# fatimp/SIFT3D

Hardware: AMD Instinct MI355X
Metric: Mvoxel/s detect+describe (float32 volume resident in HBM) (higher is better)
Workload: dtype f32; 1 GPU; 512x512x512 float32 lattice-blob volume, detect+describe, default parameters (sigma0 1.6, sigma_n 1.15, 3 levels/octave); parallelism=single GPU

## Files before the change

### include/sift3d_amd.h

```cpp
#ifndef SIFT3D_AMD_H
#define SIFT3D_AMD_H

#include <stddef.h>
#include <stdint.h>

#include "sift3d/imtypes.h"

#ifdef __cplusplus
extern "C" {
#endif

#define SIFT3D_AMD_API __attribute__((visibility("default")))


SIFT3D_AMD_API int
sift3d_amd_detect_keypoints_device(sift3d_detector *det, const float *d_volume,
                                   int nx, int ny, int nz, double ux, double uy,
                                   double uz, sift3d_keypoint_store *store);

SIFT3D_AMD_API int
sift3d_amd_image_set_units(sift3d_image *im, double ux, double uy, double uz);

SIFT3D_AMD_API int
sift3d_amd_detector_set_cuboid_extrema(sift3d_detector *det, int on);
// ... 813 lines not shown
    int32_t level;
    uint32_t row1;
    double sd;
} sift3d_hip_kp;

SIFT3D_AMD_API int
sift3d_hip_describe(const sift3d_hip_level *d_levels, const sift3d_hip_kp *d_kp,
                    uint32_t n, float *d_hist, void *stream);

SIFT3D_AMD_API size_t sift3d_hip_describe_wlut_floats(int nlevels);
SIFT3D_AMD_API int
sift3d_hip_describe_wlut(const sift3d_hip_level *d_levels, int nlevels, const sift3d_hip_kp *d_kp,
                         uint32_t n, float *d_hist, float *d_wlut, void *stream);
SIFT3D_AMD_API size_t sift3d_hip_describe_part_bytes(uint32_t n);
SIFT3D_AMD_API int
sift3d_hip_describe_parts(const sift3d_hip_level *d_levels, int nlevels, const sift3d_hip_kp *d_kp,
                          uint32_t n, uint32_t n_exact, float *d_hist, float *d_hist2, float *d_wlut,
                          void *d_part, void *stream);
SIFT3D_AMD_API int sift3d_hip_describe_lattice_level(float ux, float uy, float uz, double sd);
SIFT3D_AMD_API int
sift3d_hip_describe_lattice(const sift3d_hip_level *d_levels, int nlevels, const sift3d_hip_kp *d_kp,
                            uint32_t n, uint32_t n_exact, uint32_t n_lattice, float *d_hist, float *d_hist2,
                            float *d_wlut, void *d_part, void *stream);
SIFT3D_AMD_API int sift3d_hip_describe_addr32_level(const sift3d_hip_level *level, double sd);
SIFT3D_AMD_API int sift3d_hip_describe_addr32_records(const sift3d_hip_level *levels, int nlevels,
                                                      const sift3d_hip_kp *kp, uint32_t n);
SIFT3D_AMD_API int sift3d_hip_describe_addr_mode(int mode);
SIFT3D_AMD_API int
sift3d_hip_describe_lattice_a32(const sift3d_hip_level *d_levels, int nlevels, const sift3d_hip_kp *d_kp,
                                uint32_t n, uint32_t n_exact, uint32_t n_lattice, float *d_hist, float *d_hist2,
                                float *d_wlut, void *d_part, void *stream, int addr32);
SIFT3D_AMD_API int sift3d_hip_describe_rcp_check(uint32_t e_lo, uint32_t n_exp, uint64_t *mismatches,
                                                 uint32_t *first_bits, void *stream);
SIFT3D_AMD_API int
sift3d_hip_describe_clock(const float *d_wlut, int nlevels, int exact, uint64_t *cycles, uint64_t *ticks,
                          void *stream);
SIFT3D_AMD_API int
sift3d_hip_describe_wlut2(const sift3d_hip_level *d_levels, int nlevels, const sift3d_hip_kp *d_kp,
                          uint32_t n, float *d_hist, float *d_hist2, float *d_wlut, void *stream);
SIFT3D_AMD_API int
sift3d_hip_describe_ex(const sift3d_hip_level *d_levels, int nlevels, const sift3d_hip_kp *d_kp, uint32_t n,
                       uint32_t n_exact, float *d_hist, float *d_hist2, float *d_wlut, void *stream);

SIFT3D_AMD_API int sift3d_hip_slab_count(const sift3d_hip_cand *d_cand, const int32_t *d_keep, uint32_t n,
                                         int ngl, int K, int nkey, int32_t *d_cnt, void *stream);
SIFT3D_AMD_API size_t sift3d_hip_slab_pack_scratch_bytes(uint32_t n);
SIFT3D_AMD_API int sift3d_hip_slab_pack(const sift3d_hip_level *d_levels, const sift3d_hip_cand *d_cand,
                                        const int32_t *d_keep, const float *d_R, uint32_t n, int ngl,
                                        float *d_vals, void *d_recs, void *d_scratch, void *stream);
SIFT3D_AMD_API int sift3d_hip_slab_build(const void *d_all, size_t blk_bytes, size_t roff, size_t toff,
                                         int world, int nkey, const uint32_t *d_tab, uint32_t tot_k,
                                         uint32_t tot_c, void *d_out, void *stream);
typedef struct {
    size_t tot_c, tot_k;
    size_t maxc, maxk;
    size_t roff, toff, blk;
} sift3d_amd_slab_layout;
SIFT3D_AMD_API int sift3d_amd_slab_table(const void *cnt, size_t cnt_stride, int world, int nkey, uint32_t *tab,
                                         sift3d_amd_slab_layout *lay);

#define SIFT3D_HIP_FACE_FLOATS 19
SIFT3D_AMD_API int
sift3d_hip_set_mesh(const float *faces );

SIFT3D_AMD_API int
sift3d_hip_synth_lattice(float *d_dst, int nx, int ny, int nz, int z_off, uint64_t seed,
// ... 15 lines not shown
```

### profiles/describe_isa_cost.py

```python
#!/usr/bin/env python3
import argparse
import os
import re
import subprocess
import sys
import tempfile

HERE = os.path.dirname(os.path.abspath(__file__))
CSRC = os.path.join(HERE, "..", "sift3d_amd", "csrc")
RATES = os.path.join(HERE, "microbench", "valu_rate_mi355x.txt")
FLAGS = ["--offload-arch=gfx950", "-O3", "-ffp-contract=off", "-fPIC", "-std=c++17", "-fvisibility=hidden",
         "-fno-slp-vectorize", "--cuda-device-only", "-S", "-w"]
SUFFIXES = ("_e32", "_e64", "_dpp", "_sdwa", "_e64_dpp")
SALU_APART = ("s_waitcnt", "s_nop", "s_branch", "s_cbranch", "s_barrier", "s_endpgm", "s_sleep", "s_setprio")


def rates(path=RATES, waves=4):
    tab = {}
    for line in open(path):
        m = re.match(r"(\w+)\s+(\d+) waves/SIMD:.*->\s*([\d.]+) cycles", line)
        if m and int(m.group(2)) == waves:
            tab[m.group(1)] = float(m.group(3))
    return tab


def assembly(opt):
    with tempfile.TemporaryDirectory() as tmp:
        out = os.path.join(tmp, "describe.s")
        cmd = ["hipcc"] + FLAGS + ([] if opt is None else ["-DDESC_OPT=%d" % opt]) + ["sift3d_describe.hip", "-o", out]
        subprocess.run(cmd, cwd=CSRC, check=True)
        return open(out).read()


def kernel_body(text, instance):
    frag = "k_describeI" + "".join("Lb%dE" % (v.strip() == "true") for v in instance.split(",")) + "E"
    m = re.search(r"^(_Z\d+%s\w*):" % re.escape(frag), text, re.M)
    if not m:
        sys.exit("no instantiation %s in the assembly" % frag)
    end = text.index(".Lfunc_end", m.end())
    return m.group(1), text[m.end():end]


def base(op):
    for s in sorted(SUFFIXES, key=len, reverse=True):
        if op.endswith(s):
            return op[:-len(s)]
    return op


def blocks(body):
    out, cur = [], dict(label="entry", loop=None, depth=0, header=False, ops=[])
    for line in body.split("\n"):
        s = line.strip()
        m = re.match(r"(?:\.L(BB\d+_\d+)|; %bb\.(\d+)):\s*(?:;\s*(.*))?$", s)
        if m:
            out.append(cur)
            cur = dict(label=m.group(1) or "bb." + m.group(2), loop=None, depth=0, header=False, ops=[])
            note = m.group(3) or ""
            h = re.search(r"in Loop: Header=(BB\d+_\d+) Depth=(\d+)", note)
            if h:
                cur["loop"], cur["depth"] = h.group(1), int(h.group(2))
            elif "Loop Header" in note or "Parent Loop" in note:
                cur["header"] = True
            if re.search(r"This (Inner )?Loop Header: Depth=(\d+)", note):
                cur["header"], cur["loop"] = True, cur["label"]
                cur["depth"] = int(re.search(r"Depth=(\d+)", note).group(1))
            continue
        if cur["header"] and s.startswith(";"):
            h = re.search(r"This (?:Inner )?Loop Header: Depth=(\d+)", s)
            if h:
                cur["loop"], cur["depth"] = cur["label"], int(h.group(1))
            p = re.search(r"Parent Loop (BB\d+_\d+) Depth=(\d+)", s)
            if p:
                cur.setdefault("parents", []).append(p.group(1))
            continue
        if not s or s[0] in ";." or s.endswith(":"):
            continue
        cur["ops"].append(s.split()[0])
    out.append(cur)
    return out


def census(ops, tab, default):
    c = dict(valu=0, salu=0, lds=0, vmem=0, other=0, cycles=0.0)
    for op in ops:
        if op.startswith("v_"):
            c["valu"] += 1
            c["cycles"] += tab.get(base(op), default)
        elif op.startswith(SALU_APART):
            c["other"] += 1
        elif op.startswith("s_"):
            c["salu"] += 1
        elif op.startswith("ds_"):
            c["lds"] += 1
        elif op.startswith(("global_", "buffer_", "flat_")):
            c["vmem"] += 1
        else:
            c["other"] += 1
    return c


def row(name, c):
    return "%-22s %5d %5d %5d %5d %6d %9.0f" % (name, c["valu"], c["salu"], c["lds"], c["vmem"], c["other"], c["cycles"])


def add(cs):
    return {k: sum(c[k] for c in cs) for k in cs[0]}


def main():
    ap = argparse.ArgumentParser()
    ap.add_argument("--instance", default="false,true,false", help="template arguments of the instantiation")
    ap.add_argument("--opt", type=int, default=None, help="build with -DDESC_OPT=N")
    ap.add_argument("--asm", default=None, help="read this assembly file instead of compiling")
    ap.add_argument("--all", action="store_true", help="print every basic block")
    a = ap.parse_args()
    tab = rates()
    default = tab["v_fma_f32"]
    name, body = kernel_body(open(a.asm).read() if a.asm else assembly(a.opt), a.instance)
    bl = blocks(body)
    cs = [census(b["ops"], tab, default) for b in bl]
    print("# %s" % name)
    print("# VALU priced at 4 waves/SIMD (%s); opcodes not in the table: %.2f cycles" % (os.path.basename(RATES), default))
    print("%-22s %5s %5s %5s %5s %6s %9s" % ("block (loop, depth)", "VALU", "SALU", "LDS", "VMEM", "other", "VALU cyc"))
    for b, c in zip(bl, cs):
        if a.all or len(b["ops"]) >= 20:
            print(row("%s (%s, %d)" % (b["label"], b["loop"] or "-", b["depth"]), c))
    print(row("kernel", add(cs)))
    loops = {}
    for i, b in enumerate(bl):
        if b["loop"]:
            loops.setdefault(b["loop"], []).append(i)
    with_lds = [h for h, ix in loops.items() if sum(cs[i]["lds"] for i in ix) >= 32]
    if not with_lds:
        return
    batch_loop = max(with_lds, key=lambda h: max(len(bl[i]["ops"]) for i in loops[h]))
    big = sorted(sorted(loops[batch_loop], key=lambda i: -len(bl[i]["ops"]))[:2])
    print("# steady state of a batch (loop %s)" % batch_loop)
    for k, i in enumerate(big):
        print(row("pass %d = %s" % (k, bl[i]["label"]), cs[i]))
    print(row("both passes", add([cs[i] for i in big])))
    header = next(b for b in bl if b["label"] == batch_loop)
    parents = header.get("parents", [])
    if parents:
        scan = parents[-1]
        ix = [i for i in loops.get(scan, []) if bl[i]["loop"] == scan]
        print(row("scan iteration (%s)" % scan, add([cs[i] for i in ix])))


if __name__ == "__main__":
    main()
```

### sift3d_amd/csrc/sift3d_describe.hip

```cpp
#include "sift3d_kernels_common.h"
#include "sift3d_math.h"

#include <algorithm>
#include <cmath>
#include <cstdlib>

struct FaceRec {
    float v0[3], e1[3], e2[3], t[3], q[3], e2q, idx[3];
};
static_assert(sizeof(FaceRec) == SIFT3D_HIP_FACE_FLOATS * 4, "face record layout");

__constant__ float c_face16[20 * 16];
__constant__ int c_bin_off[12];
__constant__ int c_oct_face[32];

constexpr int DQ = 256;
constexpr int HIST_USED = 800;
constexpr int HIST_LDS = 800;
constexpr int FACE_STRIDE = 20;
constexpr int RSUPER = 68;
constexpr int REC_FLOATS = 7 * RSUPER;
constexpr int rec_row(int r) { return r < 7 ? r * RSUPER : (r - 7) * RSUPER + 32; }
constexpr int rec_group(int r) { return (rec_row(r) / 4) % 16; }
constexpr bool rec_groups_distinct()
// ... 13 lines not shown
}

#ifdef SIFT3D_AMD_DIAG
#define DESC_ABLATE_ARG , int ablate
#define DESC_ABLATE(bit) (ablate & (bit))
__device__ unsigned long long g_desc_voxels;
#else
#define DESC_ABLATE_ARG
#define DESC_ABLATE(bit) false
#endif

__device__ __forceinline__ void wave_sync()
{
    __builtin_amdgcn_fence(__ATOMIC_RELEASE, "wavefront");
    __builtin_amdgcn_wave_barrier();
    __builtin_amdgcn_fence(__ATOMIC_ACQUIRE, "wavefront");
}

__device__ __forceinline__ float quad_fmac(float acc, float x)
{
    asm("v_fmac_f32_dpp %0, %1, %1 quad_perm:[3,0,0,0] row_mask:0xf bank_mask:0xf bound_ctrl:1"
        : "+v"(acc)
        : "v"(x));
    return acc;
}

__device__ __forceinline__ float desc_rcp(float x)
{
    const float r = __builtin_amdgcn_rcpf(x);
    return __builtin_fmaf(r, __builtin_fmaf(-x, r, 1.0f), r);
}

__device__ __forceinline__ bool face_eval(const float4 *__restrict__ fr, float rx, float ry, float rz,
                                          float &xb, float &yb, float &zb, int &fi)
{
    const float4 A0 = fr[0], A1 = fr[1], A2 = fr[2], A3 = fr[3];
    const float px = ry * A1.y - rz * A1.x;
    const float py = rz * A0.w - rx * A1.y;
    const float pz = rx * A1.x - ry * A0.w;
    const float det = A0.x * px + A0.y * py + A0.z * pz;
    const float di = 1.0f / det;
    yb = di * (A1.z * px + A1.w * py + A2.x * pz);
    zb = di * (rx * A2.y + ry * A2.z + rz * A2.w);
    xb = 1.0f - yb - zb;
    const float kk = A3.x * di;
    fi = __float_as_int(A3.y);
    return !(fabsf(det) < 1.1920928955078125e-06f) &&
           !(xb < -1.1920928955078125e-06f || yb < -1.1920928955078125e-06f ||
             zb < -1.1920928955078125e-06f || kk < 0);
}

__device__ __forceinline__ int icos_guess(float rx, float ry, float rz)
{
    const float g = 1.6180339887f, g2 = 2.6180339887f;
    const float ax = fabsf(rx), ay = fabsf(ry), az = fabsf(rz);
    const float t1 = ax + g2 * ay - g * az;
    const float t2 = ay + g2 * az - g * ax;
    const float t3 = az + g2 * ax - g * ay;
    const int n1 = t1 < 0.0f, n2 = t2 < 0.0f, n3 = t3 < 0.0f;
    const int cls = n1 + (1 - n1) * (2 * n2 + (1 - n2) * 3 * n3);
    return cls * 8 + (int)(rx < 0.0f) + 2 * (int)(ry < 0.0f) + 4 * (int)(rz < 0.0f);
}

constexpr int WL_STRIDE = 4096, WL_HEAD = 4;
constexpr int WL_COUNTERS = 16;

__global__ __launch_bounds__(256) void k_desc_wlut(const sift3d_hip_level *__restrict__ levels, int nlevels,
                                                   float *__restrict__ lut)
{
    const int t = blockIdx.x;
    if (t >= nlevels)
        return;
    if (t == 0 && threadIdx.x < WL_COUNTERS)
        reinterpret_cast<uint32_t *>(lut + (size_t)nlevels * WL_STRIDE)[threadIdx.x] = 0u;
    const sift3d_hip_level L = levels[t];
    float *tab = lut + (size_t)t * WL_STRIDE;
    const float sigma = (float)(L.sd * 7.071067812);
    const float rad = (float)(2.0 * (double)sigma);
    const float rad2 = rad * rad, sig2 = sigma * sigma;
    int e;
    const float mant = frexpf(L.ux, &e);
    const float u2 = L.ux * L.ux;
    const bool ok = L.ux == L.uy && L.ux == L.uz && mant == 0.5f &&
                    rad2 / u2 < (float)(WL_STRIDE - WL_HEAD - 1) && u2 * (float)WL_STRIDE < 16777216.0f;
    if (threadIdx.x == 0) {
        tab[0] = ok ? 1.0f : 0.0f;
        tab[1] = 0.0f;
        tab[2] = __int_as_float((int)(__double_as_longlong(L.sd) & 0xffffffffll));
        tab[3] = __int_as_float((int)(__double_as_longlong(L.sd) >> 32));
    }
    if (!ok)
        return;
    for (int k = threadIdx.x; k < WL_STRIDE - WL_HEAD; k += 256) {
        const float sq = (float)k * u2;
        const float arg = -0.5f * sq / sig2;
        tab[WL_HEAD + k] = arg >= -150.0f ? s3d_expf(arg) : 0.0f;
    }
}

#ifndef DESC_OPT
#define DESC_OPT 495
#endif

constexpr int DWAVES = 4;
constexpr int DPARTS = 4;

template <bool EXACT, bool LATTICE = false, bool A64 = false>
__global__ __launch_bounds__(64 * DWAVES) void k_describe(const sift3d_hip_level *__restrict__ levels,
                                                 const sift3d_hip_kp *__restrict__ kps, uint32_t first,
                                                 uint32_t n,
                                                 float *__restrict__ out, float *__restrict__ out2,
                                                 const float *__restrict__ wlut,
                                                 uint32_t *__restrict__ work, float *__restrict__ part,
                                                 uint32_t *__restrict__ done DESC_ABLATE_ARG)
{
    __shared__ float hist_[DWAVES][2 * HIST_LDS];
    __shared__ __attribute__((aligned(16))) float rec_[DWAVES][REC_FLOATS];
    __shared__ int queue_[DWAVES][DQ];
    __shared__ __attribute__((aligned(16))) float sface[20 * FACE_STRIDE];
    __shared__ int soct[32];
    __shared__ uint64_t sexp[32];
    const int wv = __builtin_amdgcn_readfirstlane((int)(threadIdx.x >> 6));
    const int lane = threadIdx.x & 63;
    float *const hist = hist_[wv];
    float *const rec = rec_[wv];
    const uint32_t rec_m0 = (uint32_t)__builtin_amdgcn_readfirstlane((int)lds_addr(rec));
    const uint32_t hist_m0 = (uint32_t)__builtin_amdgcn_readfirstlane((int)lds_addr(hist));
    int *const queue = queue_[wv];
    for (int i = threadIdx.x; i < 20 * 16; i += 64 * DWAVES)
        sface[(i >> 4) * FACE_STRIDE + (i & 15)] = c_face16[i];
    if (threadIdx.x < 32) {
        soct[threadIdx.x] = c_oct_face[threadIdx.x];
        if (!LATTICE)
            sexp[threadIdx.x] = s3d_exp2_tab[threadIdx.x];
    }
    __syncthreads();
    const bool probe = work && blockIdx.x == 0 && threadIdx.x == 0;
    long long probe_c0 = 0, probe_w0 = 0;
    if (probe) {
        probe_c0 = clock64();
        probe_w0 = wall_clock64();
    }
    const bool split = !EXACT && part != nullptr;
    for (bool first_pass = true;; first_pass = false) {
    uint32_t item;
    if (work) {
        uint32_t t = 0;
        if (lane == 0)
            t = atomicAdd(work, 1u);
        item = (uint32_t)__builtin_amdgcn_readfirstlane((int)t);
    } else {
        if (!first_pass)
            break;
        item = blockIdx.x * DWAVES + wv;
    }
    const uint32_t ki = first + (split ? item / DPARTS : item);
    const int pp = split ? (int)(item % DPARTS) : 0;
    if (ki >= n)
        break;
    static_assert(2 * HIST_LDS == 25 * 64, "histogram clear: 25 whole-wave stores");
#define Z4(o) "ds_write_addtid_b32 %0 offset:" #o "\n\tds_write_addtid_b32 %0 offset:" #o "+256\n\t" \
              "ds_write_addtid_b32 %0 offset:" #o "+512\n\tds_write_addtid_b32 %0 offset:" #o "+768\n\t"
    asm volatile("s_mov_b32 m0, %1\n\ts_nop 0\n\t" Z4(0) Z4(1024) Z4(2048) Z4(3072) Z4(4096) Z4(5120)
                 "ds_write_addtid_b32 %0 offset:6144" ::"v"(0.0f), "s"(hist_m0) : "m0", "memory");
#undef Z4
// ... 198 lines not shown
        float *bin_ = reinterpret_cast<float *>(reinterpret_cast<char *>(hist) + (mb_[(u) & 3] + coff4)); \
        float old_ = 0.0f;                                                                    \
        if (!DESC_ABLATE(1))                                                                  \
            old_ = *bin_;                                                                     \
        SB();                                                                                 \
        { __VA_ARGS__ }                                                                       \
        SB();                                                                                 \
        if (!DESC_ABLATE(1))                                                                  \
            *bin_ = COMMIT_ADD(old_, xv_[(u) & 3]);                     \
        if (((u) & 3) == 3) {                                                                 \
            cb4 = nb4;                                                                        \
            cx4 = nx4;                                                                        \
        }                                                                                     \
        SB();                                                                                 \
    }
#endif
#define CHAIN_B()                                                                             \
    if (EXACT) {                                                                              \
        COMMIT_BEGIN(coff_b);                                                                 \
        ROUND(0, ) ROUND(1, ) ROUND(2, ) ROUND(3, ) ROUND(4, ) ROUND(5, ) ROUND(6, ) ROUND(7, ) \
        ROUND(8, ) ROUND(9, ) ROUND(10, ) ROUND(11, ) ROUND(12, ) ROUND(13, ) ROUND(14, ) ROUND(15, ) \
    }
    auto batch = [&](int cnt, const float *cv, int pk, uint32_t nstart, int ncnt) {
#ifdef SIFT3D_AMD_DIAG
        diag_voxels += (unsigned)cnt;
#endif
        if (DESC_ABLATE(2)) { prefetch(nstart, ncnt); return; }
        int x, y, z;
        float dx, dy, dz, kx, ky, kz, vbx, vby, vbz, gx, gy, gz, rx, ry, rz, m2;
        float t1, t2, t3, px, py, pz, det, di, kk;
        float4 A0, A1, A2, A3;
        int f0;
        bool live = false, found = false;
        int fidx = 0;
        float b0 = 0.f, b1 = 0.f, b2 = 0.f;
        commit_write(0);
        {
            COMMIT_BEGIN(coff_a);
            ROUND(0, if (LATTICE && (DESC_OPT & 8)) {
                         dx = (float)pwi * L.ux; dy = (float)pwj * L.uy; dz = (float)pwl * L.uz;
                         KEEP(dy); KEEP(dz);
                     } else {
                         x = B.xs + (int)((uint32_t)pk & xmask); y = B.ys + (int)(((uint32_t)pk >> xsh) & ymask);
                         z = B.zs + (int)((uint32_t)pk >> ysh);
                         dx = ((float)x - K.cx) * L.ux;
                     }
                     KEEP(dx);)
            ROUND(1, if (!(LATTICE && (DESC_OPT & 8))) {
                         dy = ((float)y - K.cy) * L.uy; dz = ((float)z - K.cz) * L.uz; KEEP(dy); KEEP(dz);
                     }
                     gx = 0.5f * (cv[0] - cv[1]); gy = 0.5f * (cv[2] - cv[3]); gz = 0.5f * (cv[4] - cv[5]);)
            ROUND(2, gx *= iux; gy *= iuy; gz *= iuz;
                     gx = gx * cv[6]; gy = gy * cv[6]; gz = gz * cv[6];)
            ROUND(3, kx = R[0] * dx + R[3] * dy + R[6] * dz; ky = R[1] * dx + R[4] * dy + R[7] * dz; KEEP(kx); KEEP(ky);)
            ROUND(4, kz = R[2] * dx + R[5] * dy + R[8] * dz;
                     vbx = (kx + half_w) * bin_f; vby = (ky + half_w) * bin_f; vbz = (kz + half_w) * bin_f;
                     KEEP(vbx); KEEP(vby); KEEP(vbz);)
            ROUND(5, rx = R[0] * gx + R[3] * gy + R[6] * gz; ry = R[1] * gx + R[4] * gy + R[7] * gz;)
            ROUND(6, rz = R[2] * gx + R[5] * gy + R[8] * gz; m2 = rx * rx + ry * ry + rz * rz;
                     live = lane < cnt && !(m2 < 1.1920928955078125e-06f);)
#if DESC_OPT & 2
            ROUND(7, const float g = 1.6180339887f, g2 = 2.6180339887f;
                     const float ax_ = fabsf(rx), ay_ = fabsf(ry), az_ = fabsf(rz);
                     t1 = __builtin_fmaf(g2, ay_, __builtin_fmaf(-g, az_, ax_));
                     t2 = __builtin_fmaf(g2, az_, __builtin_fmaf(-g, ax_, ay_));
                     t3 = __builtin_fmaf(g2, ax_, __builtin_fmaf(-g, ay_, az_));)
#else
            ROUND(7, const float g = 1.6180339887f, g2 = 2.6180339887f;
                     const float ax_ = fabsf(rx), ay_ = fabsf(ry), az_ = fabsf(rz);
                     t1 = ax_ + g2 * ay_ - g * az_; t2 = ay_ + g2 * az_ - g * ax_; t3 = az_ + g2 * ax_ - g * ay_;)
#endif
            ROUND(8, const int n1 = t1 < 0.0f, n2 = t2 < 0.0f, n3 = t3 < 0.0f;
                     const int cls = n1 + (1 - n1) * (2 * n2 + (1 - n2) * 3 * n3);
                     f0 = soct[cls * 8 + (int)(rx < 0.0f) + 2 * (int)(ry < 0.0f) + 4 * (int)(rz < 0.0f)];)
            ROUND(9, const float4 *fr = reinterpret_cast<const float4 *>(sface + f0 * FACE_STRIDE);
                     A0 = fr[0]; A1 = fr[1]; A2 = fr[2]; A3 = fr[3];)
            ROUND(10, px = ry * A1.y - rz * A1.x; py = rz * A0.w - rx * A1.y; pz = rx * A1.x - ry * A0.w;)
            ROUND(11, det = A0.x * px + A0.y * py + A0.z * pz; di = EXACT || !(DESC_OPT & 256) ? 1.0f / det : desc_rcp(det);)
            ROUND(12, b1 = di * (A1.z * px + A1.w * py + A2.x * pz);)
            ROUND(13, b2 = di * (rx * A2.y + ry * A2.z + rz * A2.w); b0 = 1.0f - b1 - b2;)
            ROUND(14, kk = A3.x * di; fidx = __float_as_int(A3.y);
                      found = !(fabsf(det) < 1.1920928955078125e-06f) &&
                              !(b0 < -1.1920928955078125e-06f || b1 < -1.1920928955078125e-06f ||
                                b2 < -1.1920928955078125e-06f || kk < 0) &&
                              fminf(b0, fminf(b1, b2)) > 2e-5f;)
            ROUND(15, )
        }
        CHAIN_B();
        if (__builtin_expect(__ballot(live && !found) != 0ull, 0)) {
            bool open = live && !found;
#pragma unroll 1
            for (int f = 0; f < 20; f++) {
                float xb, yb, zb;
                int fi;
                const bool hit = face_eval(reinterpret_cast<const float4 *>(sface + f * FACE_STRIDE), rx,
                                           ry, rz, xb, yb, zb, fi);
                if (open && hit) {
                    b0 = xb; b1 = yb; b2 = zb; fidx = fi;
                    found = true;
                    open = false;
                }
                if (__ballot(open) == 0ull)
                    break;
            }
        }
        commit_write(1);
        {
            COMMIT_BEGIN(coff_a);
            int nx_, ny_, nzl_, qv_;
            gfloat_p np_;
            uint32_t no_;
            float mag, fx, fy, fz;
            int ix, iy, iz, cell4;
            float ax[2], ay[2], az[2], fld[14];
            ROUND(0, qv_ = queue[(nstart + lane) & (DQ - 1)];)
            ROUND(1, ppk = lane < ncnt ? qv_ : ppk;
                     nx_ = B.xs + (int)((uint32_t)ppk & xmask); ny_ = B.ys + (int)(((uint32_t)ppk >> xsh) & ymask);
                     if (A32) {
                         no_ = 4u * ((uint32_t)ppk & xmask) + ys4 * (((uint32_t)ppk >> xsh) & ymask) +
                               zs4 * ((uint32_t)ppk >> ysh);
                     } else {
                         nzl_ = B.zs + (int)((uint32_t)ppk >> ysh) - L.z_off;
                         np_ = gdata + ((uint64_t)zs32 * (uint32_t)nzl_ + (uint32_t)(nx_ + (int)ys32 * ny_));
                     })
            ROUND(2, if (A32) {
                         pv[0] = GLD32(gb_c + 4, no_); pv[1] = GLD32(gb_c - 4, no_);
                         pv[2] = GLD32(gb_yp, no_); pv[3] = GLD32(gb_ym, no_);
                     } else {
                         pv[0] = np_[1]; pv[1] = *(np_ - 1); pv[2] = np_[ys32]; pv[3] = *(np_ - ys32);
                     })
            ROUND(3, if (A32) {
                         pv[4] = GLD32(gb_zp, no_); pv[5] = GLD32(gb_zm, no_);
                     } else {
                         pv[4] = np_[zs32]; pv[5] = *(np_ - zs32);
                     }
                     const int i = nx_ - icx; const int j = ny_ - icy; const int l = B.zs + (int)((uint32_t)ppk >> ysh) - icz;
                     pv[6] = A32 ? GLD32(wsrc_b, (4u * (uint32_t)(i * i + j * j + l * l)) & (uint32_t)wmask)
                                 : wsrc[(i * i + j * j + l * l) & wmask];
                     if (LATTICE && (DESC_OPT & 8)) { pwi = i; pwj = j; pwl = l; })
#if DESC_OPT & 2
            ROUND(4, mag = EXACT ? sqrtf(m2) : __builtin_amdgcn_sqrtf(m2);
                     mag = live && found ? mag : 0.0f;)
#else
            ROUND(4, mag = sqrtf(m2); mag = live && found ? mag : 0.0f;)
#endif
            ROUND(5, fx = vbx - floorf(vbx); fy = vby - floorf(vby); fz = vbz - floorf(vbz);
                     ix = (int)vbx; iy = (int)vby; iz = (int)vbz;)
            ROUND(6, const bool lx = ix >= 3; const bool ly = iy >= 3; const bool lz = iz >= 3;
                     ax[0] = lx ? 0.0f : 1.0f - fx; ax[1] = lx ? 1.0f - fx : fx;
                     ay[0] = ly ? 0.0f : 1.0f - fy; ay[1] = ly ? 1.0f - fy : fy;
                     az[0] = lz ? 0.0f : 1.0f - fz; az[1] = lz ? 1.0f - fz : fz;)
            ROUND(7, _Pragma("unroll") for (int c = 0; c < 4; c++)
                         fld[c] = mag * (ax[(c >> 2) & 1] * ay[(c >> 1) & 1] * az[c & 1]);)
            ROUND(8, _Pragma("unroll") for (int c = 4; c < 8; c++)
                         fld[c] = mag * (ax[(c >> 2) & 1] * ay[(c >> 1) & 1] * az[c & 1]);)
            ROUND(9, cell4 = 4 * (min(max(ix, 0), 2) + 4 * min(max(iy, 0), 2) + 16 * min(max(iz, 0), 2));
                     const bool ok = live && found;
                     fld[8] = ok ? b0 : 0.0f; fld[9] = ok ? b1 : 0.0f; fld[10] = ok ? b2 : 0.0f;)
            ROUND(10, _Pragma("unroll") for (int j = 0; j < 3; j++)
                          fld[11 + j] = __int_as_float(4 * ((fidx >> (10 * j)) & 1023) + cell4);)
            ROUND(11, _Pragma("unroll") for (int i = 0; i < 4; i++) {
                          const auto r = __builtin_amdgcn_permlane32_swap(__float_as_uint(fld[i]), __float_as_uint(fld[7 + i]), false, false);
                          rp[0][i] = __uint_as_float(r[0]); rp[1][i] = __uint_as_float(r[1]); })
            ROUND(12, _Pragma("unroll") for (int i = 4; i < 7; i++) {
                          const auto r = __builtin_amdgcn_permlane32_swap(__float_as_uint(fld[i]), __float_as_uint(fld[7 + i]), false, false);
                          rp[0][i] = __uint_as_float(r[0]); rp[1][i] = __uint_as_float(r[1]); })
            ROUND(13, )
            ROUND(14, )
            ROUND(15, )
        }
        CHAIN_B();
        prefetch_weight();
    };
    auto commit_tail = [&](int pass) {
        commit_write(pass);
        {
            COMMIT_BEGIN(coff_a);
            ROUND(0, ) ROUND(1, ) ROUND(2, ) ROUND(3, ) ROUND(4, ) ROUND(5, ) ROUND(6, ) ROUND(7, )
            ROUND(8, ) ROUND(9, ) ROUND(10, ) ROUND(11, ) ROUND(12, ) ROUND(13, ) ROUND(14, ) ROUND(15, )
        }
        CHAIN_B();
    };

    float ortho = 0.0f;
#pragma unroll
    for (int a = 0; a < 3; a++)
#pragma unroll
        for (int b = a; b < 3; b++)
            ortho = fmaxf(ortho, fabsf(R[a] * R[b] + R[3 + a] * R[3 + b] + R[6 + a] * R[6 + b] - (a == b ? 1.0f : 0.0f)));
    const bool cube_ok = ortho <= 1e-4f;
    const float cube_x = cube_ok ? half_w * (fabsf(R[0]) + fabsf(R[1]) + fabsf(R[2])) * 1.001f : rad * 1.001f;
    const float cube_y = cube_ok ? half_w * (fabsf(R[3]) + fabsf(R[4]) + fabsf(R[5])) * 1.001f : rad * 1.001f;
    const float cube_z = cube_ok ? half_w * (fabsf(R[6]) + fabsf(R[7]) + fabsf(R[8])) * 1.001f : rad * 1.001f;
// ... 187 lines not shown
                el = el < trunc ? el : trunc;
            hist[i] = el;
        }
        wave_sync();
    }
    for (int i = lane; i < 768; i += 64) {
        const float v = hist[c_bin_off[i % 12] + i / 12];
        out[(size_t)orow * 768 + i] = v;
        if (out2)
            out2[(size_t)orow * 768 + i] = v;
    }
    wave_sync();
    }
    if (probe) {
        unsigned long long *slot =
            reinterpret_cast<unsigned long long *>(work - (EXACT ? 0 : LATTICE ? 2 : 1) + (EXACT ? 4 : 8));
        slot[0] = (unsigned long long)(clock64() - probe_c0);
        slot[1] = (unsigned long long)(wall_clock64() - probe_w0);
    }
}

__constant__ int c_face_vert[20];

constexpr int DB_TX = 64, DB_TY = 4;

__device__ __forceinline__ void dense_bin_one(const float *sface, const int *soct, const int *svert, float gx,
                                              float gy, float gz, float &w0, float &w1, float &w2, int &vid)
{
    const float m2 = gx * gx + gy * gy + gz * gz;
    w0 = 0.0f; w1 = 0.0f; w2 = 0.0f; vid = 0;
    if (m2 < 1.1920928955078125e-06f)
        return;
    float b0, b1, b2;
    int fi, f = soct[icos_guess(gx, gy, gz)];
    bool found = face_eval(reinterpret_cast<const float4 *>(sface + f * FACE_STRIDE), gx, gy, gz, b0, b1, b2, fi) &&
                 fminf(b0, fminf(b1, b2)) > 2e-5f;
    if (!found) {
        for (f = 0; f < 20; f++)
            if (face_eval(reinterpret_cast<const float4 *>(sface + f * FACE_STRIDE), gx, gy, gz, b0, b1, b2, fi)) {
                found = true;
                break;
            }
        if (!found)
            return;
    }
    const float mag = sqrtf(m2);
    w0 = mag * b0; w1 = mag * b1; w2 = mag * b2;
    vid = svert[f];
}

__device__ __forceinline__ float dense_pick(int c, int vid, float w0, float w1, float w2)
{
    return c == (vid & 15) ? w0 : c == ((vid >> 4) & 15) ? w1 : c == (vid >> 8) ? w2 : 0.0f;
}

template <int V>
__global__ __launch_bounds__(DB_TX * DB_TY) void k_dense_bin(const float *__restrict__ src, float *__restrict__ out,
                                                             int nx, int ny, int nz, float iux, float iuy, float iuz)
{
    __shared__ __attribute__((aligned(16))) float sface[20 * FACE_STRIDE];
    __shared__ int soct[32], svert[20];
    const int tid = threadIdx.x + DB_TX * threadIdx.y;
    for (int i = tid; i < 20 * 16; i += DB_TX * DB_TY)
        sface[(i >> 4) * FACE_STRIDE + (i & 15)] = c_face16[i];
    if (tid < 32)
        soct[tid] = c_oct_face[tid];
    if (tid < 20)
// ... 370 lines not shown
                for (int b = 0; b < 3; b++)
                    if (a != b)
                        adj[idx[f * 3 + a]][idx[f * 3 + b]] = true;
        for (int v = 0; v < 12; v++)
            colour[v] = -1;
        int v = 0;
        while (v >= 0 && v < 12) {
            int c = colour[v] + 1;
            for (; c < 4; c++) {
                bool clash = false;
                for (int u = 0; u < v; u++)
                    clash = clash || (adj[v][u] && colour[u] == c);
                if (!clash)
                    break;
            }
            if (c < 4) {
                colour[v++] = c;
            } else {
                colour[v--] = -1;
            }
        }
        if (v < 0) {
            snprintf(g_err, sizeof(g_err), "sift3d_hip_set_mesh: vertex graph is not 4-colourable");
            return SIFT3D_FAILURE;
        }
        static const int shift[4] = { 0, 8, 18, 26 };
        int rank = 0;
        for (int c = 0; c < 4; c++)
            for (int u = 0; u < 12; u++)
                if (colour[u] == c)
                    binoff[u] = 64 * rank++ + shift[c];
    }
    for (int f = 0; f < 20; f++) {
        const int packed = binoff[idx[f * 3]] | (binoff[idx[f * 3 + 1]] << 10) |
                           (binoff[idx[f * 3 + 2]] << 20);
        memcpy(f16 + f * 16 + 13, &packed, sizeof(int));
    }
    int oct[32];
    {
        const float g = 1.6180339887f;
        const float rep[4][3] = { { 1.0f, 1.0f, 1.0f },
                                  { g / 3.0f, 0.05f, (2.0f * g + 1.0f) / 3.0f },
                                  { (2.0f * g + 1.0f) / 3.0f, g / 3.0f, 0.05f },
                                  { 0.05f, (2.0f * g + 1.0f) / 3.0f, g / 3.0f } };
        for (int c = 0; c < 4; c++)
            for (int o = 0; o < 8; o++) {
                const float r[3] = { (o & 1) ? -rep[c][0] : rep[c][0], (o & 2) ? -rep[c][1] : rep[c][1],
                                     (o & 4) ? -rep[c][2] : rep[c][2] };
                int hit = -1;
                for (int f = 0; f < 20 && hit < 0; f++)
                    if (host_face_pass(f16, f, r))
                        hit = f;
                if (hit < 0) {
                    snprintf(g_err, sizeof(g_err), "sift3d_hip_set_mesh: no face holds a probe direction");
                    return SIFT3D_FAILURE;
                }
                oct[c * 8 + o] = hit;
            }
    }
    HIPCHK(hipMemcpyToSymbol(HIP_SYMBOL(c_bin_off), binoff, sizeof(binoff)));
    HIPCHK(hipMemcpyToSymbol(HIP_SYMBOL(c_face16), f16, sizeof(f16)));
    HIPCHK(hipMemcpyToSymbol(HIP_SYMBOL(c_oct_face), oct, sizeof(oct)));
    int vert[20];
    {
        float P[20][3][3];
        for (int f = 0; f < 20; f++)
            for (int k = 0; k < 3; k++) {
                const float *r = faces + f * SIFT3D_HIP_FACE_FLOATS;
                P[f][0][k] = r[k];
// ... 124 lines not shown
    for (uint64_t i = blockIdx.x * (uint64_t)blockDim.x + threadIdx.x; i < total;
         i += (uint64_t)gridDim.x * blockDim.x) {
        const uint32_t bits = (uint32_t)(i & 1) << 31 | (e_lo + (uint32_t)(i >> 24)) << 23 | ((uint32_t)(i >> 1) & 0x7fffffu);
        const float x = __uint_as_float(bits);
        if (__float_as_uint(desc_rcp(x)) != __float_as_uint(1.0f / x)) {
            bad++;
            first = bits < first ? bits : first;
        }
    }
    if (bad) {
        atomicAdd(out, bad);
        atomicMin(out + 1, first);
    }
}

int sift3d_hip_describe_rcp_check(uint32_t e_lo, uint32_t n_exp, uint64_t *mismatches, uint32_t *first_bits,
                                  void *stream)
{
    if (!mismatches || !first_bits || e_lo < 1 || n_exp < 1 || e_lo + n_exp > 255)
        return launch_fail("sift3d_hip_describe_rcp_check", "exponents outside 1 .. 254");
    unsigned long long h[2] = { 0ull, ~0ull }, *d = nullptr;
    HIPCHK(hipMalloc(&d, sizeof(h)));
    hipError_t e = hipMemcpyAsync(d, h, sizeof(h), hipMemcpyHostToDevice, (hipStream_t)stream);
    if (e == hipSuccess) {
        hipLaunchKernelGGL(k_desc_rcp_check, dim3(4096), dim3(256), 0, (hipStream_t)stream, e_lo, n_exp, d);
        e = hipGetLastError();
    }
    if (e == hipSuccess)
        e = hipMemcpyAsync(h, d, sizeof(h), hipMemcpyDeviceToHost, (hipStream_t)stream);
    const hipError_t e2 = hipStreamSynchronize((hipStream_t)stream);
    (void)hipFree(d);
    if (e != hipSuccess || e2 != hipSuccess)
        return fail("k_desc_rcp_check", e != hipSuccess ? e : e2, __FILE__, __LINE__);
    *mismatches = h[0];
    *first_bits = (uint32_t)h[1];
    return SIFT3D_SUCCESS;
}

static int describe_launch(const sift3d_hip_level *d_levels, int nlevels, const sift3d_hip_kp *d_kp, uint32_t n,
                           uint32_t n_exact, uint32_t n_lattice, float *d_hist, float *d_hist2,
                           const float *d_wlut, void *d_part, void *stream, int addr32 = 0)
{
    const bool a64 = g_desc_addr_mode == 1 ? false : g_desc_addr_mode == 2 ? true : !addr32;
    if (n_exact > n)
        n_exact = n;
    if (!(DESC_OPT & 8) || !d_wlut)
        n_lattice = 0;
    if (n_lattice > n - n_exact)
        return launch_fail("sift3d_hip_describe", "more lattice records than fast records");
#ifdef SIFT3D_AMD_DIAG
    static int ablate = getenv("SIFT3D_AMD_DESC_ABLATE") ? atoi(getenv("SIFT3D_AMD_DESC_ABLATE")) : 0;
#define DESC_ABLATE_PASS , ablate
#else
#define DESC_ABLATE_PASS
#endif
    uint32_t *work = d_wlut ? reinterpret_cast<uint32_t *>(const_cast<float *>(d_wlut) + (size_t)nlevels * WL_STRIDE)
                            : nullptr;
    if (n_exact) {
        hipLaunchKernelGGL((a64 ? k_describe<true, false, true> : k_describe<true, false, false>),
                           dim3(describe_grid(n_exact, work != nullptr)), dim3(64 * DWAVES), 0,
                           (hipStream_t)stream, d_levels, d_kp, 0u, n_exact, d_hist, d_hist2, d_wlut,
                           work, (float *)nullptr, (uint32_t *)nullptr DESC_ABLATE_PASS);
        LAUNCH_CHECK();
    }
    if (n > n_exact) {
        const uint32_t nf = n - n_exact;
// ... 228 lines not shown
```

### sift3d_amd/hip.py

```python
import collections
import ctypes as C

import numpy as np

from . import _native

MAX_TAPS = 65
FACE_FLOATS = 19


class FirArgs(C.Structure):
    _fields_ = [("src", C.c_void_p), ("dst", C.c_void_p), ("nx", C.c_int), ("ny", C.c_int),
                ("nz", C.c_int), ("axis", C.c_int), ("width", C.c_int),
                ("taps", C.POINTER(C.c_float)), ("unit_factor", C.c_float), ("n_glob", C.c_int),
                ("off", C.c_int), ("z_lo", C.c_int), ("z_hi", C.c_int), ("variant", C.c_int)]


class ExtremaLevel(C.Structure):
    _fields_ = [("prev", C.c_void_p), ("cur", C.c_void_p), ("next", C.c_void_p),
                ("d_absmax", C.c_void_p), ("z_lo", C.c_int), ("z_hi", C.c_int), ("tag", C.c_int)]


class ExtremaOct(C.Structure):
    _fields_ = [("d_g", C.POINTER(C.c_void_p)), ("nx", C.c_int), ("ny", C.c_int), ("nz", C.c_int),
# ... 2360 lines not shown

def describe_addr_mode(mode):
    f = lib().sift3d_hip_describe_addr_mode
    f.restype, f.argtypes = C.c_int, [C.c_int]
    return f(int(mode))


def describe_addr32_level(nx, ny, nz, uz, sd):
    f = lib().sift3d_hip_describe_addr32_level
    f.restype, f.argtypes = C.c_int, [C.POINTER(Level), C.c_double]
    L = Level(None, nx, ny, nz, 0, nz, 1.0, 1.0, uz, 0, sd)
    return f(C.byref(L), float(sd))


def describe_addr32_records(levels, kps):
    f = lib().sift3d_hip_describe_addr32_records
    f.restype, f.argtypes = C.c_int, [C.POINTER(Level), C.c_int, C.c_void_p, C.c_uint32]
    tab = (Level * len(levels))(*[Level(None, nx, ny, nz, 0, nz, 1.0, 1.0, uz, 0, sd)
                                  for nx, ny, nz, uz, sd in levels])
    kps = np.ascontiguousarray(kps, KP_DTYPE)
    return f(tab, len(levels), kps.ctypes.data, len(kps))


def describe_rcp_check(e_lo, n_exp):
    f = lib().sift3d_hip_describe_rcp_check
    f.restype, f.argtypes = C.c_int, [C.c_uint32, C.c_uint32, C.POINTER(C.c_uint64), C.POINTER(C.c_uint32),
                                      C.c_void_p]
    bad, first = C.c_uint64(0), C.c_uint32(0)
    _check(f(int(e_lo), int(n_exp), C.byref(bad), C.byref(first), current_stream()),
           "sift3d_hip_describe_rcp_check")
    return int(bad.value), int(first.value)



def _dev_bytes(t, need, what, name, dtype=None):
    _tensor(t, "%s: %s must be a contiguous %sCUDA tensor of >= %d bytes" % (what, name, dtype + " " if dtype else "",
                                                                             need), dtype=dtype)
    if t.numel() * t.element_size() < need:
        raise ValueError("%s: %s holds fewer than %d bytes" % (what, name, need))
    return t.data_ptr()


def slab_count(cand, keep, n, ngl, K, nkey, cnt):
    what, n = "slab_count", int(n)
    _tensor(cnt, "slab_count: cnt must be a contiguous int32 CUDA tensor [2 * nkey]", shape=(2 * max(int(nkey), 0),),
            dtype="int32")
    _check(lib().sift3d_hip_slab_count(_dev_bytes(cand, CAND_DTYPE.itemsize * n, what, "cand", "uint8"),
                                       _dev_bytes(keep, 4 * n, what, "keep", "int32"), n, int(ngl), int(K),
                                       int(nkey), cnt.data_ptr(), current_stream()), "sift3d_hip_slab_count")


def slab_pack_scratch_bytes(n):
    return int(lib().sift3d_hip_slab_pack_scratch_bytes(int(n)))


def slab_pack(d_levels, cand, keep, R, n, ngl, vals, recs, scratch):
    what, n = "slab_pack", int(n)
    _tensor(d_levels, "slab_pack: d_levels must be the uint8 CUDA tensor of level_table()", dtype="uint8")
    _dev_bytes(recs, 0, what, "recs", "uint8")
    if d_levels.numel() % LEVEL_DTYPE.itemsize or recs.numel() % SLAB_REC_DTYPE.itemsize:
        raise ValueError("slab_pack: d_levels / recs must hold whole records")
    _check(lib().sift3d_hip_slab_pack(d_levels.data_ptr(), _dev_bytes(cand, CAND_DTYPE.itemsize * n, what, "cand",
                                                                      "uint8"),
                                      _dev_bytes(keep, 4 * n, what, "keep", "int32"),
                                      _dev_bytes(R, 36 * n, what, "R", "float32"), n, int(ngl),
                                      _dev_bytes(vals, 4 * n, what, "vals", "float32"), recs.data_ptr(),
# ... 46 lines not shown
```

Measured before the change: 4472 Mvoxel/s.

## Trim describe inner-loop ALU: bitpacked octant lookup, unpacked bin offsets, native fract

Raises the default DESC_OPT to enable four micro-optimisations in the descriptor gradient loop. The octant/class face lookup now packs sign bits with alignbit into a 64-entry LDS table of byte offsets. Face bin offsets are stored as three precomputed words instead of one 10-bit-packed int. floor-based fraction is replaced with v_fract, and a redundant barycentric negativity test is dropped. This cuts VALU work per sample at the cost of a slightly larger shared table and a face-record layout change. A fract equivalence checker and ISA-profile tooling are added to validate the change.

```diff
diff --git a/include/sift3d_amd.h b/include/sift3d_amd.h
--- a/include/sift3d_amd.h
+++ b/include/sift3d_amd.h
@@ -869,6 +869,8 @@
                                 float *d_wlut, void *d_part, void *stream, int addr32);
 SIFT3D_AMD_API int sift3d_hip_describe_rcp_check(uint32_t e_lo, uint32_t n_exp, uint64_t *mismatches,
                                                  uint32_t *first_bits, void *stream);
+SIFT3D_AMD_API int sift3d_hip_describe_fract_check(uint32_t n_bits, uint64_t *mismatches, uint32_t *first_bits,
+                                                   void *stream);
 SIFT3D_AMD_API int
 sift3d_hip_describe_clock(const float *d_wlut, int nlevels, int exact, uint64_t *cycles, uint64_t *ticks,
                           void *stream);
diff --git a/profiles/describe_isa_cost.py b/profiles/describe_isa_cost.py
--- a/profiles/describe_isa_cost.py
+++ b/profiles/describe_isa_cost.py
@@ -49,13 +49,13 @@
 
 
 def blocks(body):
-    out, cur = [], dict(label="entry", loop=None, depth=0, header=False, ops=[])
+    out, cur = [], dict(label="entry", loop=None, depth=0, header=False, ops=[], last="")
     for line in body.split("\n"):
         s = line.strip()
         m = re.match(r"(?:\.L(BB\d+_\d+)|; %bb\.(\d+)):\s*(?:;\s*(.*))?$", s)
         if m:
             out.append(cur)
-            cur = dict(label=m.group(1) or "bb." + m.group(2), loop=None, depth=0, header=False, ops=[])
+            cur = dict(label=m.group(1) or "bb." + m.group(2), loop=None, depth=0, header=False, ops=[], last="")
             note = m.group(3) or ""
             h = re.search(r"in Loop: Header=(BB\d+_\d+) Depth=(\d+)", note)
             if h:
@@ -77,6 +77,7 @@
         if not s or s[0] in ";." or s.endswith(":"):
             continue
         cur["ops"].append(s.split()[0])
+        cur["last"] = s
     out.append(cur)
     return out
 
@@ -134,7 +135,7 @@
     with_lds = [h for h, ix in loops.items() if sum(cs[i]["lds"] for i in ix) >= 32]
     if not with_lds:
         return
-    batch_loop = max(with_lds, key=lambda h: max(len(bl[i]["ops"]) for i in loops[h]))
+    batch_loop = max(with_lds, key=lambda h: (bl[loops[h][0]]["depth"], max(len(bl[i]["ops"]) for i in loops[h])))
     big = sorted(sorted(loops[batch_loop], key=lambda i: -len(bl[i]["ops"]))[:2])
     print("# steady state of a batch (loop %s)" % batch_loop)
     for k, i in enumerate(big):
@@ -146,6 +147,15 @@
         scan = parents[-1]
         ix = [i for i in loops.get(scan, []) if bl[i]["loop"] == scan]
         print(row("scan iteration (%s)" % scan, add([cs[i] for i in ix])))
+        order = {b["label"]: i for i, b in enumerate(bl)}
+        side = []
+        for i in ix:
+            t = re.match(r"s_branch\s+\.L(BB\d+_\d+)$", bl[i]["last"])
+            if t and bl[i - 1]["loop"] != scan and order.get(t.group(1), i) < i:
+                side.append(i)
+        print(row("  straight path", add([cs[i] for i in ix if i not in side])))
+        for i in side:
+            print(row("  out of line: %s" % bl[i]["label"], cs[i]))
 
 
 if __name__ == "__main__":
diff --git a/sift3d_amd/csrc/sift3d_describe.hip b/sift3d_amd/csrc/sift3d_describe.hip
--- a/sift3d_amd/csrc/sift3d_describe.hip
+++ b/sift3d_amd/csrc/sift3d_describe.hip
@@ -69,7 +69,7 @@
 }
 
 __device__ __forceinline__ bool face_eval(const float4 *__restrict__ fr, float rx, float ry, float rz,
-                                          float &xb, float &yb, float &zb, int &fi)
+                                          float &xb, float &yb, float &zb, int3 &fi)
 {
     const float4 A0 = fr[0], A1 = fr[1], A2 = fr[2], A3 = fr[3];
     const float px = ry * A1.y - rz * A1.x;
@@ -81,7 +81,7 @@
     zb = di * (rx * A2.y + ry * A2.z + rz * A2.w);
     xb = 1.0f - yb - zb;
     const float kk = A3.x * di;
-    fi = __float_as_int(A3.y);
+    fi = make_int3(__float_as_int(A3.y), __float_as_int(A3.z), __float_as_int(A3.w));
     return !(fabsf(det) < 1.1920928955078125e-06f) &&
            !(xb < -1.1920928955078125e-06f || yb < -1.1920928955078125e-06f ||
              zb < -1.1920928955078125e-06f || kk < 0);
@@ -136,8 +136,9 @@
 }
 
 #ifndef DESC_OPT
-#define DESC_OPT 495
-#endif
+#define DESC_OPT 8175
+#endif
+#define FACE_BYTES(f) ((f) * (FACE_STRIDE * 4))
 
 constexpr int DWAVES = 4;
 constexpr int DPARTS = 4;
@@ -155,7 +156,11 @@
     __shared__ __attribute__((aligned(16))) float rec_[DWAVES][REC_FLOATS];
     __shared__ int queue_[DWAVES][DQ];
     __shared__ __attribute__((aligned(16))) float sface[20 * FACE_STRIDE];
+#if DESC_OPT & 512
+    __shared__ int soct64[64];
+#else
     __shared__ int soct[32];
+#endif
     __shared__ uint64_t sexp[32];
     const int wv = __builtin_amdgcn_readfirstlane((int)(threadIdx.x >> 6));
     const int lane = threadIdx.x & 63;
@@ -166,8 +171,17 @@
     int *const queue = queue_[wv];
     for (int i = threadIdx.x; i < 20 * 16; i += 64 * DWAVES)
         sface[(i >> 4) * FACE_STRIDE + (i & 15)] = c_face16[i];
+#if DESC_OPT & 512
+    if (threadIdx.x < 64) {
+        const int i = threadIdx.x;
+        const int cls = (i & 8) ? 1 : (i & 16) ? 2 : (i & 32) ? 3 : 0;
+        soct64[i] = FACE_BYTES(c_oct_face[cls * 8 + (i & 7)]);
+    }
+#endif
     if (threadIdx.x < 32) {
+#if !(DESC_OPT & 512)
         soct[threadIdx.x] = c_oct_face[threadIdx.x];
+#endif
         if (!LATTICE)
             sexp[threadIdx.x] = s3d_exp2_tab[threadIdx.x];
     }
@@ -432,7 +446,7 @@
         float4 A0, A1, A2, A3;
         int f0;
         bool live = false, found = false;
-        int fidx = 0;
+        int3 fidx = make_int3(0, 0, 0);
         float b0 = 0.f, b1 = 0.f, b2 = 0.f;
         commit_write(0);
         {
@@ -470,20 +484,40 @@
                      const float ax_ = fabsf(rx), ay_ = fabsf(ry), az_ = fabsf(rz);
                      t1 = ax_ + g2 * ay_ - g * az_; t2 = ay_ + g2 * az_ - g * ax_; t3 = az_ + g2 * ax_ - g * ay_;)
 #endif
+#if DESC_OPT & 512
+            ROUND(8, uint32_t gi = __float_as_uint(t3) >> 31;
+                     gi = __builtin_amdgcn_alignbit(gi, __float_as_uint(t2), 31);
+                     gi = __builtin_amdgcn_alignbit(gi, __float_as_uint(t1), 31);
+                     gi = __builtin_amdgcn_alignbit(gi, __float_as_uint(rz), 31);
+                     gi = __builtin_amdgcn_alignbit(gi, __float_as_uint(ry), 31);
+                     gi = __builtin_amdgcn_alignbit(gi, __float_as_uint(rx), 31);
+                     f0 = soct64[gi];)
+            ROUND(9, const float4 *fr = reinterpret_cast<const float4 *>(reinterpret_cast<const char *>(sface) + f0);
+                     A0 = fr[0]; A1 = fr[1]; A2 = fr[2]; A3 = fr[3];)
+#else
             ROUND(8, const int n1 = t1 < 0.0f, n2 = t2 < 0.0f, n3 = t3 < 0.0f;
                      const int cls = n1 + (1 - n1) * (2 * n2 + (1 - n2) * 3 * n3);
                      f0 = soct[cls * 8 + (int)(rx < 0.0f) + 2 * (int)(ry < 0.0f) + 4 * (int)(rz < 0.0f)];)
             ROUND(9, const float4 *fr = reinterpret_cast<const float4 *>(sface + f0 * FACE_STRIDE);
                      A0 = fr[0]; A1 = fr[1]; A2 = fr[2]; A3 = fr[3];)
+#endif
             ROUND(10, px = ry * A1.y - rz * A1.x; py = rz * A0.w - rx * A1.y; pz = rx * A1.x - ry * A0.w;)
             ROUND(11, det = A0.x * px + A0.y * py + A0.z * pz; di = EXACT || !(DESC_OPT & 256) ? 1.0f / det : desc_rcp(det);)
             ROUND(12, b1 = di * (A1.z * px + A1.w * py + A2.x * pz);)
             ROUND(13, b2 = di * (rx * A2.y + ry * A2.z + rz * A2.w); b0 = 1.0f - b1 - b2;)
-            ROUND(14, kk = A3.x * di; fidx = __float_as_int(A3.y);
+#if DESC_OPT & 4096
+            ROUND(14, kk = A3.x * di;
+                      fidx = make_int3(__float_as_int(A3.y), __float_as_int(A3.z), __float_as_int(A3.w));
+                      found = !(fabsf(det) < 1.1920928955078125e-06f) && !(kk < 0) &&
+                              fminf(b0, fminf(b1, b2)) > 2e-5f;)
+#else
+            ROUND(14, kk = A3.x * di;
+                      fidx = make_int3(__float_as_int(A3.y), __float_as_int(A3.z), __float_as_int(A3.w));
                       found = !(fabsf(det) < 1.1920928955078125e-06f) &&
                               !(b0 < -1.1920928955078125e-06f || b1 < -1.1920928955078125e-06f ||
                                 b2 < -1.1920928955078125e-06f || kk < 0) &&
                               fminf(b0, fminf(b1, b2)) > 2e-5f;)
+#endif
             ROUND(15, )
         }
         CHAIN_B();
@@ -492,7 +526,7 @@
 #pragma unroll 1
             for (int f = 0; f < 20; f++) {
                 float xb, yb, zb;
-                int fi;
+                int3 fi;
                 const bool hit = face_eval(reinterpret_cast<const float4 *>(sface + f * FACE_STRIDE), rx,
                                            ry, rz, xb, yb, zb, fi);
                 if (open && hit) {
@@ -544,8 +578,14 @@
 #else
             ROUND(4, mag = sqrtf(m2); mag = live && found ? mag : 0.0f;)
 #endif
+#if DESC_OPT & 2048
+            ROUND(5, fx = __builtin_amdgcn_fractf(vbx); fy = __builtin_amdgcn_fractf(vby);
+                     fz = __builtin_amdgcn_fractf(vbz);
+                     ix = (int)vbx; iy = (int)vby; iz = (int)vbz;)
+#else
             ROUND(5, fx = vbx - floorf(vbx); fy = vby - floorf(vby); fz = vbz - floorf(vbz);
                      ix = (int)vbx; iy = (int)vby; iz = (int)vbz;)
+#endif
             ROUND(6, const bool lx = ix >= 3; const bool ly = iy >= 3; const bool lz = iz >= 3;
                      ax[0] = lx ? 0.0f : 1.0f - fx; ax[1] = lx ? 1.0f - fx : fx;
                      ay[0] = ly ? 0.0f : 1.0f - fy; ay[1] = ly ? 1.0f - fy : fy;
@@ -557,8 +597,13 @@
             ROUND(9, cell4 = 4 * (min(max(ix, 0), 2) + 4 * min(max(iy, 0), 2) + 16 * min(max(iz, 0), 2));
                      const bool ok = live && found;
                      fld[8] = ok ? b0 : 0.0f; fld[9] = ok ? b1 : 0.0f; fld[10] = ok ? b2 : 0.0f;)
+#if DESC_OPT & 1024
+            ROUND(10, fld[11] = __int_as_float(fidx.x + cell4); fld[12] = __int_as_float(fidx.y + cell4);
+                      fld[13] = __int_as_float(fidx.z + cell4);)
+#else
             ROUND(10, _Pragma("unroll") for (int j = 0; j < 3; j++)
-                          fld[11 + j] = __int_as_float(4 * ((fidx >> (10 * j)) & 1023) + cell4);)
+                          fld[11 + j] = __int_as_float(4 * ((fidx.x >> (10 * j)) & 1023) + cell4);)
+#endif
             ROUND(11, _Pragma("unroll") for (int i = 0; i < 4; i++) {
                           const auto r = __builtin_amdgcn_permlane32_swap(__float_as_uint(fld[i]), __float_as_uint(fld[7 + i]), false, false);
                           rp[0][i] = __uint_as_float(r[0]); rp[1][i] = __uint_as_float(r[1]); })
@@ -812,7 +857,8 @@
     if (m2 < 1.1920928955078125e-06f)
         return;
     float b0, b1, b2;
-    int fi, f = soct[icos_guess(gx, gy, gz)];
+    int3 fi;
+    int f = soct[icos_guess(gx, gy, gz)];
     bool found = face_eval(reinterpret_cast<const float4 *>(sface + f * FACE_STRIDE), gx, gy, gz, b0, b1, b2, fi) &&
                  fminf(b0, fminf(b1, b2)) > 2e-5f;
     if (!found) {
@@ -1249,9 +1295,14 @@
                     binoff[u] = 64 * rank++ + shift[c];
     }
     for (int f = 0; f < 20; f++) {
+#if DESC_OPT & 1024
+        const int off4[3] = { 4 * binoff[idx[f * 3]], 4 * binoff[idx[f * 3 + 1]], 4 * binoff[idx[f * 3 + 2]] };
+        memcpy(f16 + f * 16 + 13, off4, sizeof(off4));
+#else
         const int packed = binoff[idx[f * 3]] | (binoff[idx[f * 3 + 1]] << 10) |
                            (binoff[idx[f * 3 + 2]] << 20);
         memcpy(f16 + f * 16 + 13, &packed, sizeof(int));
+#endif
     }
     int oct[32];
     {
@@ -1442,6 +1493,45 @@
     (void)hipFree(d);
     if (e != hipSuccess || e2 != hipSuccess)
         return fail("k_desc_rcp_check", e != hipSuccess ? e : e2, __FILE__, __LINE__);
+    *mismatches = h[0];
+    *first_bits = (uint32_t)h[1];
+    return SIFT3D_SUCCESS;
+}
+
+__global__ __launch_bounds__(256) void k_desc_fract_check(uint32_t n_bits, unsigned long long *out)
+{
+    unsigned long long bad = 0, first = ~0ull;
+    for (uint64_t i = blockIdx.x * (uint64_t)blockDim.x + threadIdx.x; i < n_bits;
+         i += (uint64_t)gridDim.x * blockDim.x) {
+        const float x = __uint_as_float((uint32_t)i);
+        if (__float_as_uint(__builtin_amdgcn_fractf(x)) != __float_as_uint(x - floorf(x))) {
+            bad++;
+            first = i < first ? i : first;
+        }
+    }
+    if (bad) {
+        atomicAdd(out, bad);
+        atomicMin(out + 1, first);
+    }
+}
+
+int sift3d_hip_describe_fract_check(uint32_t n_bits, uint64_t *mismatches, uint32_t *first_bits, void *stream)
+{
+    if (!mismatches || !first_bits || n_bits < 1 || n_bits > 0x7f800000u)
+        return launch_fail("sift3d_hip_describe_fract_check", "bit patterns outside the finite non-negative floats");
+    unsigned long long h[2] = { 0ull, ~0ull }, *d = nullptr;
+    HIPCHK(hipMalloc(&d, sizeof(h)));
+    hipError_t e = hipMemcpyAsync(d, h, sizeof(h), hipMemcpyHostToDevice, (hipStream_t)stream);
+    if (e == hipSuccess) {
+        hipLaunchKernelGGL(k_desc_fract_check, dim3(4096), dim3(256), 0, (hipStream_t)stream, n_bits, d);
+        e = hipGetLastError();
+    }
+    if (e == hipSuccess)
+        e = hipMemcpyAsync(h, d, sizeof(h), hipMemcpyDeviceToHost, (hipStream_t)stream);
+    const hipError_t e2 = hipStreamSynchronize((hipStream_t)stream);
+    (void)hipFree(d);
+    if (e != hipSuccess || e2 != hipSuccess)
+        return fail("k_desc_fract_check", e != hipSuccess ? e : e2, __FILE__, __LINE__);
     *mismatches = h[0];
     *first_bits = (uint32_t)h[1];
     return SIFT3D_SUCCESS;
diff --git a/sift3d_amd/hip.py b/sift3d_amd/hip.py
--- a/sift3d_amd/hip.py
+++ b/sift3d_amd/hip.py
@@ -2416,6 +2416,14 @@
     return int(bad.value), int(first.value)
 
 
+def describe_fract_check(n_bits):
+    f = lib().sift3d_hip_describe_fract_check
+    f.restype, f.argtypes = C.c_int, [C.c_uint32, C.POINTER(C.c_uint64), C.POINTER(C.c_uint32), C.c_void_p]
+    bad, first = C.c_uint64(0), C.c_uint32(0)
+    _check(f(int(n_bits), C.byref(bad), C.byref(first), current_stream()), "sift3d_hip_describe_fract_check")
+    return int(bad.value), int(first.value)
+
+
 
 def _dev_bytes(t, need, what, name, dtype=None):
     _tensor(t, "%s: %s must be a contiguous %sCUDA tensor of >= %d bytes" % (what, name, dtype + " " if dtype else "",
```

After: 4524 Mvoxel/s (median of 6 runs). 1.2% higher.
